# Jiahao-Ma/VFA

Hardware: AMD Instinct MI355X
Metric: voxels aggregated/sec (7 views->BEV grid) (higher is better)
Workload: dtype f32; 1 GPU; multiviewc_200x200x1; cameras_per_rank=7, cameras_total=7, channels=256, rccl_ranks=1, parallelism=single GPU

## Files before the change

vfa_amd/csrc/vfa_integral.hip:

```cpp
#include <hip/hip_runtime.h>
#include <stdint.h>

#include "../../include/vfa_hip.h"
#include "vfa_geom.h"
#include "vfa_split.h"

namespace {
using namespace vfa_dev;

constexpr int kMaxMaps = 4;
constexpr int kChunk = 32;

struct MapDesc {
    const float *feat;
    float *out;
    const float *scale;
    const float *shift;
    int H, W;
    unsigned row_blocks;
    unsigned long long col_vecs;
    unsigned *absmax;
};
struct MapArgs {
    MapDesc m[kMaxMaps];
    int n_maps, n_views, C;
};

template <bool AFFINE>
__global__ __launch_bounds__(kWave) void rows_batched_kernel(MapArgs a)
{
    __shared__ __align__(16) float tile[kWave][kChunk + 1];
    const int lane = threadIdx.x;
    unsigned b = blockIdx.x;
    int mi = 0;
    while (mi + 1 < a.n_maps && b >= a.m[mi].row_blocks) { b -= a.m[mi].row_blocks; ++mi; }
    const MapDesc &m = a.m[mi];
    const int H = m.H, W = m.W, C = a.C, cblocks = C / kWave;
    const int y = (int)(b % (unsigned)H);
    const unsigned rest = b / (unsigned)H;
    const int c0 = (int)(rest % (unsigned)cblocks) * kWave, v = (int)(rest / (unsigned)cblocks);
    const size_t plane = (size_t)H * W;
    const float *src = m.feat + ((size_t)v * C + c0) * plane + (size_t)y * W;
    float *dst = m.out + (((size_t)v * (H + 2) + (y + 1)) * (W + 2)) * C + c0;
    dst[lane] = 0.0f;
    dst[(size_t)(W + 1) * C + lane] = 0.0f;
    float sa = 1.0f, sb = 0.0f;
    if (AFFINE) {
        sa = m.scale[(size_t)v * C + c0 + lane];
        sb = m.shift[(size_t)v * C + c0 + lane];
    }
    auto act = [&](float x) {
        if (!AFFINE) return x;
        float t = x * sa;
        t = t + sb;
        return (t < 0.0f) ? 0.0f : t;
    };
    const int q = lane & 7, cq = lane & 15;
    double acc = 0.0;
    unsigned amax = 0u;
    for (int x0 = 0; x0 < W; x0 += kChunk) {
        const int nx = min(kChunk, W - x0);
        if (4 * q < nx) {
            for (int r = lane >> 3; r < kWave; r += 8) {
                const float4 t = *reinterpret_cast<const float4 *>(src + (size_t)r * plane + x0 + 4 * q);
                tile[r][4 * q + 0] = t.x; tile[r][4 * q + 1] = t.y; tile[r][4 * q + 2] = t.z; tile[r][4 * q + 3] = t.w;
            }
        }
        __syncthreads();
        for (int k = 0; k < nx; ++k) {
            const float f = act(tile[lane][k]);
            amax = max(amax, __float_as_uint(f) & 0x7fffffffu);
            acc += (double)f;
            tile[lane][k] = (float)acc;
        }
        __syncthreads();
        for (int k = lane >> 4; k < nx; k += 4) {
            const float4 t = make_float4(tile[4 * cq + 0][k], tile[4 * cq + 1][k], tile[4 * cq + 2][k], tile[4 * cq + 3][k]);
            *reinterpret_cast<float4 *>(dst + (size_t)(x0 + k + 1) * C + 4 * cq) = t;
        }
        __syncthreads();
    }
    if (m.absmax) {
        amax = wave_max_u32(amax);
        if (lane == 0) m.absmax[b] = amax;
    }
}

template <bool AFFINE>
__global__ __launch_bounds__(kWave) void rows_hwc_kernel(MapArgs a)
{
    const int lane = threadIdx.x;
    unsigned b = blockIdx.x;
    int mi = 0;
    while (mi + 1 < a.n_maps && b >= a.m[mi].row_blocks) { b -= a.m[mi].row_blocks; ++mi; }
    const MapDesc &m = a.m[mi];
    const int H = m.H, W = m.W, C = a.C, cblocks = C / kWave;
    const int y = (int)(b % (unsigned)H);
    const unsigned rest = b / (unsigned)H;
    const int c0 = (int)(rest % (unsigned)cblocks) * kWave, v = (int)(rest / (unsigned)cblocks);
    const float *src = m.feat + (((size_t)v * H + y) * W) * C + c0 + lane;
    float *dst = m.out + (((size_t)v * (H + 2) + (y + 1)) * (W + 2)) * C + c0 + lane;
    dst[0] = 0.0f;
    dst[(size_t)(W + 1) * C] = 0.0f;
    float sa = 1.0f, sb = 0.0f;
    if (AFFINE) {
        sa = m.scale[(size_t)v * C + c0 + lane];
        sb = m.shift[(size_t)v * C + c0 + lane];
    }
    auto act = [&](float x) {
        if (!AFFINE) return x;
        float t = x * sa;
        t = t + sb;
        return (t < 0.0f) ? 0.0f : t;
    };
    constexpr int U = 8;
    double acc = 0.0;
    unsigned amax = 0u;
    int x = 0;
    for (; x + U <= W; x += U) {
        float t[U];
#pragma unroll
        for (int k = 0; k < U; ++k) t[k] = src[(size_t)(x + k) * C];
#pragma unroll
        for (int k = 0; k < U; ++k) {
            const float f = act(t[k]);
            amax = max(amax, __float_as_uint(f) & 0x7fffffffu);
            acc += (double)f;
            dst[(size_t)(x + k + 1) * C] = (float)acc;
        }
    }
    for (; x < W; ++x) {
        const float f = act(src[(size_t)x * C]);
        amax = max(amax, __float_as_uint(f) & 0x7fffffffu);
        acc += (double)f;
        dst[(size_t)(x + 1) * C] = (float)acc;
    }
    if (m.absmax) {
        amax = wave_max_u32(amax);
        if (lane == 0) m.absmax[b] = amax;
    }
}

__global__ __launch_bounds__(256) void cols_batched_kernel(MapArgs a, unsigned long long total)
{
    unsigned long long i = (unsigned long long)blockIdx.x * 256 + threadIdx.x;
    if (i >= total) return;
    i = total - 1 - i;
    int mi = 0;
    while (mi + 1 < a.n_maps && i >= a.m[mi].col_vecs) { i -= a.m[mi].col_vecs; ++mi; }
    const MapDesc &m = a.m[mi];
    const int H = m.H;
    const size_t row_vecs = (size_t)(m.W + 2) * a.C / 4;
    const size_t v = i / row_vecs, r = i % row_vecs;
    float4 *p = reinterpret_cast<float4 *>(m.out) + v * (size_t)(H + 2) * row_vecs + r;
    const float4 zero = make_float4(0.f, 0.f, 0.f, 0.f);
    p[0] = zero;
    p[(size_t)(H + 1) * row_vecs] = zero;
    p += row_vecs;
    double a0 = 0.0, a1 = 0.0, a2 = 0.0, a3 = 0.0;
    auto step = [&](float4 &t) {
        a0 += (double)t.x; t.x = (float)a0;
        a1 += (double)t.y; t.y = (float)a1;
        a2 += (double)t.z; t.z = (float)a2;
        a3 += (double)t.w; t.w = (float)a3;
    };
    constexpr int U = 8;
    int y = 0;
    for (; y + U <= H; y += U) {
        float4 t[U];
#pragma unroll
        for (int k = 0; k < U; ++k) t[k] = p[(size_t)(y + k) * row_vecs];
#pragma unroll
        for (int k = 0; k < U; ++k) {
            step(t[k]);
            p[(size_t)(y + k) * row_vecs] = t[k];
        }
    }
    for (; y < H; ++y) {
        float4 t = p[(size_t)y * row_vecs];
        step(t);
        p[(size_t)y * row_vecs] = t;
    }
}

constexpr int kOpRows = 32, kOpCols = 32, kOpCh = 16, kOpThreads = kOpRows * kOpCh;
constexpr int kOpRowPitch = kOpCols * kOpCh + 16;
struct OnePassArgs {
    MapDesc m[kMaxMaps];
    unsigned unit_end[kMaxMaps];
    int split[kMaxMaps];
    int n_maps, n_views, C;
};
__device__ __forceinline__ void lds_barrier()
{
    asm volatile("s_waitcnt lgkmcnt(0)" ::: "memory");
    __builtin_amdgcn_s_barrier();
    asm volatile("" ::: "memory");
}
template <bool AFFINE>
__global__ __launch_bounds__(kOpThreads, 4) void integral_onepass_kernel(OnePassArgs a)
{
    extern __shared__ __align__(16) unsigned char op_lds[];
    float *tile = reinterpret_cast<float *>(op_lds);
    double *colacc = reinterpret_cast<double *>(op_lds + kOpRows * kOpRowPitch * 4);
    const int tid = threadIdx.x;
    unsigned u = blockIdx.x;
    int mi = 0;
    while (mi + 1 < a.n_maps && u >= a.unit_end[mi]) ++mi;
    if (mi > 0) u -= a.unit_end[mi - 1];
    const MapDesc &m = a.m[mi];
    const int H = m.H, W = m.W, C = a.C, cblocks = C / kOpCh;
    const int split = a.split[mi], part = split ? (int)(u & 1u) : 0;
    if (split) u >>= 1;
    const int v = (int)(u / (unsigned)cblocks), cb = (int)(u % (unsigned)cblocks), c0 = cb * kOpCh;
    const int r = tid >> 4, c = tid & 15;
    const size_t plane = (size_t)H * W;
    float *out_v = m.out + (size_t)v * (H + 2) * (W + 2) * C + c0;
    const int n_strips = (W + kOpCols - 1) / kOpCols;
    const int s_first = part ? split : 0, s_last = (split && !part) ? split : n_strips;
    const int xa = s_first * kOpCols, xb = min(W, s_last * kOpCols);
    {
        float *o = out_v + c;
        const int pa = part ? xa + 1 : 0, pb = (split && !part) ? xb + 1 : W + 2;
        for (int x = pa + r; x < pb; x += kOpRows) { o[(size_t)x * C] = 0.0f; o[((size_t)(H + 1) * (W + 2) + x) * C] = 0.0f; }
        for (int y = r; y < H; y += kOpRows) {
            if (!part) o[(size_t)(y + 1) * (W + 2) * C] = 0.0f;
            if (!split || part) o[((size_t)(y + 1) * (W + 2) + W + 1) * C] = 0.0f;
        }
    }
    for (int i = tid; i < (xb - xa) * kOpCh; i += kOpThreads) colacc[i] = 0.0;
    float sa = 1.0f, sb = 0.0f;
    if (AFFINE) { sa = m.scale[(size_t)v * C + c0 + c]; sb = m.shift[(size_t)v * C + c0 + c]; }
    auto act = [&](float x) {
        if (!AFFINE) return x;
        float t = x * sa;
        t = t + sb;
        return (t < 0.0f) ? 0.0f : t;
    };
    unsigned amax = 0u;
    auto load_strip = [&](float4 (&buf)[kOpCols / 4], int y0, int x0) {
        {
            const int x4 = tid & 7;
#pragma unroll
            for (int j = 0; j < kOpCols / 4; ++j) {
                const int line = (tid & ~63) + 8 * j + ((tid & 63) >> 3), row = line >> 4, ch = line & 15;
                buf[j] = *reinterpret_cast<const float4 *>(m.feat + ((size_t)v * C + c0 + ch) * plane + (size_t)min(y0 + row, H - 1) * W +
                                                           min(x0 + 4 * x4, W - 4));
            }
        }
    };
    float4 cur[kOpCols / 4];
    load_strip(cur, 0, 0);
    __syncthreads();
    bool stores_behind = false;
    for (int y0 = 0; y0 < H; y0 += kOpRows) {
        const int rows = min(kOpRows, H - y0);
        double racc = 0.0;
        for (int s = 0; s < s_last; ++s) {
            const int x0 = s * kOpCols, nx = min(kOpCols, W - x0);
            const bool carry_only = s < s_first;
            const bool last_strip = s + 1 == s_last;
            const bool more = !last_strip || y0 + kOpRows < H;
            if (stores_behind) __builtin_amdgcn_s_waitcnt(0x0f78);
            else __builtin_amdgcn_s_waitcnt(0x0f70);
            float *trow = tile + r * kOpRowPitch + c;
            {
                float *raw = tile;
#pragma unroll
                for (int j = 0; j < kOpCols / 4; ++j) {
                    float *p = raw + ((tid & ~63) + 8 * j + ((tid & 63) >> 3)) * 33 + 4 * (tid & 7);
                    p[0] = cur[j].x; p[1] = cur[j].y; p[2] = cur[j].z; p[3] = cur[j].w;
                }
#pragma unroll
                for (int j = 0; j < kOpCols / 4; ++j)
                    cur[j] = make_float4(raw[tid * 33 + 4 * j], raw[tid * 33 + 4 * j + 1], raw[tid * 33 + 4 * j + 2], raw[tid * 33 + 4 * j + 3]);
            }
            auto raw_of = [&](int k) {
                const float4 q = cur[k / 4];
                return (k & 3) == 0 ? q.x : (k & 3) == 1 ? q.y : (k & 3) == 2 ? q.z : q.w;
            };
            if (carry_only) {
                if (r < rows) {
#pragma unroll
                    for (int k = 0; k < kOpCols; ++k) racc += (double)act(raw_of(k));
                }
                if (more) load_strip(cur, last_strip ? y0 + kOpRows : y0, last_strip ? 0 : x0 + kOpCols);
                stores_behind = false;
                continue;
            }
            if (r < rows) {
                if (nx == kOpCols) {
#pragma unroll
                    for (int k = 0; k < kOpCols; ++k) {
                        const float f = act(raw_of(k));
                        amax = max(amax, __float_as_uint(f) & 0x7fffffffu);
                        racc += (double)f;
                        trow[k * kOpCh] = (float)racc;
                    }
                } else {
#pragma unroll
                    for (int k = 0; k < kOpCols; ++k) {
                        if (k < nx) {
                            const float f = act(raw_of(k));
                            amax = max(amax, __float_as_uint(f) & 0x7fffffffu);
                            racc += (double)f;
                            trow[k * kOpCh] = (float)racc;
                        }
                    }
                }
            }
            if (more) load_strip(cur, last_strip ? y0 + kOpRows : y0, last_strip ? 0 : x0 + kOpCols);
            lds_barrier();
            if (r < nx) {
                double acc = colacc[(x0 - xa + r) * kOpCh + c];
                float *tcol = tile + r * kOpCh + c;
                if (rows == kOpRows) {
#pragma unroll
                    for (int k = 0; k < kOpRows; ++k) {
                        acc += (double)tcol[k * kOpRowPitch];
                        tcol[k * kOpRowPitch] = (float)acc;
                    }
                } else {
                    for (int k = 0; k < rows; ++k) {
                        acc += (double)tcol[k * kOpRowPitch];
                        tcol[k * kOpRowPitch] = (float)acc;
                    }
                }
                colacc[(x0 - xa + r) * kOpCh + c] = acc;
            }
            lds_barrier();
#pragma unroll
            for (int j = 0; j < kOpCols / 4; ++j) {
                const int idx = tid + kOpThreads * j, row = min(idx >> 7, rows - 1), x = min((idx >> 2) & 31, nx - 1), c4 = idx & 3;
                *reinterpret_cast<float4 *>(out_v + ((size_t)(y0 + row + 1) * (W + 2) + (x0 + x + 1)) * C + 4 * c4) =
                    *reinterpret_cast<const float4 *>(tile + row * kOpRowPitch + x * kOpCh + 4 * c4);
            }
            stores_behind = more;
            lds_barrier();
        }
    }
    if (m.absmax) {
        __shared__ unsigned s_max[kOpThreads / kWave];
        amax = wave_max_u32(amax);
        if ((tid & 63) == 0) s_max[tid >> 6] = amax;
        __syncthreads();
        if (tid == 0) {
            unsigned mx = 0u;
            for (int k = 0; k < kOpThreads / kWave; ++k) mx = max(mx, s_max[k]);
            unsigned *e = m.absmax + ((size_t)v * (C / kWave) + (cb >> 2)) * H;
            const int q = 2 * (cb & 3) + part;
            for (int y = q; y < H; y += 8) e[y] = y == q ? mx : 0u;
            if (!split) for (int y = q + 1; y < H; y += 8) e[y] = 0u;
        }
    }
}

__global__ __launch_bounds__(kWave) void integral_absmax_kernel(const float *integral, unsigned *absmax, int n_views, int C, int H, int W,
                                                                unsigned units)
{
    const int lane = threadIdx.x, cblocks = (C + kWave - 1) / kWave;
    unsigned amax = 0u;
    for (unsigned b = blockIdx.x; b < units; b += gridDim.x) {
        const int y = (int)(b % (unsigned)H);
        const unsigned rest = b / (unsigned)H;
        const int c = (int)(rest % (unsigned)cblocks) * kWave + lane, v = (int)(rest / (unsigned)cblocks);
        if (c < C) {
            const float *up = integral + (((size_t)v * (H + 2) + y) * (W + 2)) * C + c, *dn = up + (size_t)(W + 2) * C;
            float u0 = up[0], d0 = dn[0];
            for (int x = 1; x <= W; ++x) {
                const float u1 = up[(size_t)x * C], d1 = dn[(size_t)x * C];
                const float f = ((d1 - u1) - d0) + u0;
                amax = max(amax, __float_as_uint(f) & 0x7fffffffu);
                u0 = u1; d0 = d1;
            }
        }
    }
    amax = wave_max_u32(amax);
    if (lane == 0) absmax[blockIdx.x] = amax;
}

bool aligned16(const void *p) { return (reinterpret_cast<uintptr_t>(p) & 15) == 0; }

}

namespace vfa_dev {
size_t feature_stats_count(int n_views, int C, int Hf)
{
    if (n_views < 0 || C <= 0 || Hf <= 0) return 0;
    return (size_t)n_views * Hf * ((C + kWave - 1) / kWave);
}
int integral_absmax_folded(const float *integral, unsigned *absmax, int n_views, int C, int Hf, int Wf, int max_entries, int *n_entries,
                               void *stream)
{
    const size_t n = feature_stats_count(n_views, C, Hf);
    if (!integral || !absmax || max_entries <= 0 || n == 0 || n >= (1ull << 31)) return VFA_ERR_BAD_ARGUMENT;
    const unsigned grid = n < (size_t)max_entries ? (unsigned)n : (unsigned)max_entries;
    hipLaunchKernelGGL(integral_absmax_kernel, dim3(grid), dim3(kWave), 0, (hipStream_t)stream, integral, absmax, n_views, C, Hf, Wf, (unsigned)n);
    *n_entries = (int)grid;
    return (int)hipGetLastError();
}

}

extern "C" {

static int integral_images_launch(const float *const *features, const float *const *scales, const float *const *shifts,
                                  float *const *integrals, unsigned *const *absmax, int n_views, int C, int n_maps, const int *feat_hw,
                                  bool hwc, void *stream)
{
    MapArgs a = {};
    a.n_maps = n_maps; a.n_views = n_views; a.C = C;
    unsigned long long row_blocks = 0, col_vecs = 0;
    for (int s = 0; s < n_maps; ++s) {
        MapDesc &m = a.m[s];
        m.feat = features[s]; m.out = integrals[s];
        m.scale = scales ? scales[s] : nullptr; m.shift = shifts ? shifts[s] : nullptr;
        m.absmax = absmax ? absmax[s] : nullptr;
        m.H = feat_hw[2 * s]; m.W = feat_hw[2 * s + 1];
        const unsigned long long rb = (unsigned long long)m.H * (C / kWave) * n_views;
        if (rb >= (1ull << 31)) return VFA_ERR_UNSUPPORTED;
        m.row_blocks = (unsigned)rb;
        m.col_vecs = (unsigned long long)n_views * (m.W + 2) * C / 4;
        row_blocks += rb; col_vecs += m.col_vecs;
    }
    if (row_blocks >= (1ull << 31) || (col_vecs + 255) / 256 >= (1ull << 31)) return VFA_ERR_UNSUPPORTED;
    hipStream_t st = (hipStream_t)stream;
    bool onepass = !hwc && C % kOpCh == 0 && C % kWave == 0 && (long long)n_views * (C / kOpCh) >= 64;
    int w_max = 0;
    for (int s = 0; s < n_maps && onepass; ++s) {
        onepass = a.m[s].H >= 8 && a.m[s].W >= 4 && (size_t)kOpRows * kOpRowPitch * 4 + (size_t)a.m[s].W * kOpCh * 8 <= 160 * 1024 - 1024;
        w_max = a.m[s].W > w_max ? a.m[s].W : w_max;
    }
    if (onepass) {
        OnePassArgs oa = {};
        oa.n_maps = n_maps; oa.n_views = n_views; oa.C = C;
        unsigned long long units = 0;
        for (int s = 0; s < n_maps; ++s) {
            oa.m[s] = a.m[s];
            const int n_strips = (a.m[s].W + kOpCols - 1) / kOpCols;
            oa.split[s] = n_strips >= 4 ? (6 * n_strips + 5) / 10 : 0;
            units += (unsigned long long)n_views * (C / kOpCh) * (oa.split[s] ? 2 : 1);
            oa.unit_end[s] = (unsigned)units;
        }
        if (units >= (1ull << 31)) return VFA_ERR_UNSUPPORTED;
        int part_max = 0;
        for (int s = 0; s < n_maps; ++s) {
            const int left = oa.split[s] * kOpCols, wide = oa.split[s] ? (left > a.m[s].W - left ? left : a.m[s].W - left) : a.m[s].W;
            part_max = wide > part_max ? wide : part_max;
        }
        const size_t lds = (size_t)kOpRows * kOpRowPitch * 4 + (size_t)part_max * kOpCh * 8;
        auto launch = [&](auto kern) {
            hipError_t e0 = hipFuncSetAttribute(reinterpret_cast<const void *>(kern), hipFuncAttributeMaxDynamicSharedMemorySize, (int)lds);
            if (e0 != hipSuccess) return (int)e0;
            hipLaunchKernelGGL(kern, dim3((unsigned)units), dim3(kOpThreads), lds, st, oa);
            return (int)hipGetLastError();
        };
        return scales ? launch(integral_onepass_kernel<true>) : launch(integral_onepass_kernel<false>);
    }
    if (hwc) {
        if (scales) hipLaunchKernelGGL((rows_hwc_kernel<true>), dim3((unsigned)row_blocks), dim3(kWave), 0, st, a);
        else hipLaunchKernelGGL((rows_hwc_kernel<false>), dim3((unsigned)row_blocks), dim3(kWave), 0, st, a);
    } else {
        if (scales) hipLaunchKernelGGL((rows_batched_kernel<true>), dim3((unsigned)row_blocks), dim3(kWave), 0, st, a);
        else hipLaunchKernelGGL((rows_batched_kernel<false>), dim3((unsigned)row_blocks), dim3(kWave), 0, st, a);
    }
    int e = (int)hipGetLastError();
    if (e) return e;
    hipLaunchKernelGGL(cols_batched_kernel, dim3((unsigned)((col_vecs + 255) / 256)), dim3(256), 0, st, a, col_vecs);
    return (int)hipGetLastError();
}

size_t vfa_feature_stats_count(int n_views, int C, int Hf) { return vfa_dev::feature_stats_count(n_views, C, Hf); }

int vfa_integral_absmax_f32(const float *integral, unsigned *absmax, int n_views, int C, int Hf, int Wf, void *stream)
{
    if (!integral || !absmax || n_views < 0 || C <= 0 || Hf <= 0 || Wf <= 0) return VFA_ERR_BAD_ARGUMENT;
    const size_t n = vfa_feature_stats_count(n_views, C, Hf);
    if (n == 0) return 0;
    if (n >= (1ull << 31)) return VFA_ERR_UNSUPPORTED;
    hipLaunchKernelGGL(integral_absmax_kernel, dim3((unsigned)n), dim3(kWave), 0, (hipStream_t)stream, integral, absmax, n_views, C, Hf, Wf,
                       (unsigned)n);
    return (int)hipGetLastError();
}

int vfa_integral_images_f32(const float *const *features, const float *const *scales, const float *const *shifts,
                            float *const *integrals, unsigned *const *absmax, int n_views, int C, int n_maps, const int *feat_hw,
                            void *stream)
{
    if (!features || !integrals || !feat_hw || n_views < 0 || C <= 0 || n_maps < 0) return VFA_ERR_BAD_ARGUMENT;
    if ((scales == nullptr) != (shifts == nullptr)) return VFA_ERR_BAD_ARGUMENT;
    for (int s = 0; s < n_maps; ++s) {
        if (feat_hw[2 * s] <= 0 || feat_hw[2 * s + 1] <= 0 || !features[s] || !integrals[s]) return VFA_ERR_BAD_ARGUMENT;
        if (scales && (!scales[s] || !shifts[s])) return VFA_ERR_BAD_ARGUMENT;
    }
    if (n_views == 0 || n_maps == 0) return 0;
    bool fast = (C % kWave == 0) && n_maps <= kMaxMaps;
    for (int s = 0; s < n_maps && fast; ++s)
        fast = (feat_hw[2 * s + 1] % 4 == 0) && aligned16(features[s]) && aligned16(integrals[s]);
    if (!fast) {
        for (int s = 0; s < n_maps; ++s) {
            const int st = scales ? vfa_affine_relu_integral_image_f32(features[s], scales[s], shifts[s], integrals[s], n_views, C,
                                                                        feat_hw[2 * s], feat_hw[2 * s + 1], stream)
                                  : vfa_integral_image_f32(features[s], integrals[s], n_views, C, feat_hw[2 * s], feat_hw[2 * s + 1], stream);
            if (st) return st;
            if (absmax && absmax[s]) {
                const int st2 = vfa_integral_absmax_f32(integrals[s], absmax[s], n_views, C, feat_hw[2 * s], feat_hw[2 * s + 1], stream);
                if (st2) return st2;
            }
        }
        return 0;
    }
    return integral_images_launch(features, scales, shifts, integrals, absmax, n_views, C, n_maps, feat_hw, false, stream);
}

int vfa_integral_images_hwc_f32(const float *const *features_hwc, const float *const *scales, const float *const *shifts,
                                float *const *integrals, unsigned *const *absmax, int n_views, int C, int n_maps, const int *feat_hw,
                                void *stream)
{
    if (!features_hwc || !integrals || !feat_hw || n_views < 0 || C <= 0 || n_maps < 0) return VFA_ERR_BAD_ARGUMENT;
    if ((scales == nullptr) != (shifts == nullptr)) return VFA_ERR_BAD_ARGUMENT;
    for (int s = 0; s < n_maps; ++s) {
        if (feat_hw[2 * s] <= 0 || feat_hw[2 * s + 1] <= 0 || !features_hwc[s] || !integrals[s]) return VFA_ERR_BAD_ARGUMENT;
        if (scales && (!scales[s] || !shifts[s])) return VFA_ERR_BAD_ARGUMENT;
    }
    if (n_views == 0 || n_maps == 0) return 0;
    if (C % kWave != 0 || n_maps > kMaxMaps) return VFA_ERR_UNSUPPORTED;
    for (int s = 0; s < n_maps; ++s)
        if (!aligned16(integrals[s])) return VFA_ERR_UNSUPPORTED;
    return integral_images_launch(features_hwc, scales, shifts, integrals, absmax, n_views, C, n_maps, feat_hw, true, stream);
}

}
```

Baseline: 1.529 billion voxels/s.

## Double-buffer strip loads via inline asm and batch LDS column scans in one-pass kernel

Restructures the one-pass integral kernel so each strip's global loads for the next strip are issued at the start, into a second register buffer, using inline asm global_load_dwordx4. This lets the loads overlap the current strip's transpose and scan work. The column scan prefetches LDS values in batches of eight, and the output stores are grouped four at a time with scheduling barriers. Occupancy hints drop from 4 to 2 blocks, and dynamic LDS is padded to at least 81KB, which appears to force lower occupancy deliberately. The trade-off is more register pressure and fewer resident blocks in exchange for more latency hiding.

Measured after the change: 1.528 billion voxels/s, median of 2. About the same (-0.1%).

```diff
diff --git a/vfa_amd/csrc/vfa_integral.hip b/vfa_amd/csrc/vfa_integral.hip
--- a/vfa_amd/csrc/vfa_integral.hip
+++ b/vfa_amd/csrc/vfa_integral.hip
@@ -184,7 +184,9 @@
 }
 
 constexpr int kOpRows = 32, kOpCols = 32, kOpCh = 16, kOpThreads = kOpRows * kOpCh;
+constexpr int kColBatch = 8;
 constexpr int kOpRowPitch = kOpCols * kOpCh + 16;
+typedef float strip_regs __attribute__((ext_vector_type(4)));
 struct OnePassArgs {
     MapDesc m[kMaxMaps];
     unsigned unit_end[kMaxMaps];
@@ -198,7 +200,7 @@
     asm volatile("" ::: "memory");
 }
 template <bool AFFINE>
-__global__ __launch_bounds__(kOpThreads, 4) void integral_onepass_kernel(OnePassArgs a)
+__global__ __launch_bounds__(kOpThreads, 2) void integral_onepass_kernel(OnePassArgs a)
 {
     extern __shared__ __align__(16) unsigned char op_lds[];
     float *tile = reinterpret_cast<float *>(op_lds);
@@ -238,31 +240,34 @@
         return (t < 0.0f) ? 0.0f : t;
     };
     unsigned amax = 0u;
-    auto load_strip = [&](float4 (&buf)[kOpCols / 4], int y0, int x0) {
+    auto load_strip = [&](strip_regs (&buf)[kOpCols / 4], int y0, int x0) {
         {
             const int x4 = tid & 7;
 #pragma unroll
             for (int j = 0; j < kOpCols / 4; ++j) {
                 const int line = (tid & ~63) + 8 * j + ((tid & 63) >> 3), row = line >> 4, ch = line & 15;
-                buf[j] = *reinterpret_cast<const float4 *>(m.feat + ((size_t)v * C + c0 + ch) * plane + (size_t)min(y0 + row, H - 1) * W +
-                                                           min(x0 + 4 * x4, W - 4));
+                const float *src = m.feat + ((size_t)v * C + c0 + ch) * plane + (size_t)min(y0 + row, H - 1) * W +
+                                   min(x0 + 4 * x4, W - 4);
+                asm volatile("global_load_dwordx4 %0, %1, off" : "=v"(buf[j]) : "v"(src) : "memory");
             }
         }
     };
-    float4 cur[kOpCols / 4];
-    load_strip(cur, 0, 0);
+    strip_regs buf_a[kOpCols / 4], buf_b[kOpCols / 4];
+    load_strip(buf_a, 0, 0);
     __syncthreads();
     bool stores_behind = false;
-    for (int y0 = 0; y0 < H; y0 += kOpRows) {
-        const int rows = min(kOpRows, H - y0);
-        double racc = 0.0;
-        for (int s = 0; s < s_last; ++s) {
+    double racc = 0.0;
+    auto strip = [&](strip_regs (&cur)[kOpCols / 4], strip_regs (&nxt)[kOpCols / 4], int y0, int s) __attribute__((always_inline)) {
+            const int rows = min(kOpRows, H - y0);
+            if (s == 0) racc = 0.0;
             const int x0 = s * kOpCols, nx = min(kOpCols, W - x0);
             const bool carry_only = s < s_first;
             const bool last_strip = s + 1 == s_last;
             const bool more = !last_strip || y0 + kOpRows < H;
             if (stores_behind) __builtin_amdgcn_s_waitcnt(0x0f78);
             else __builtin_amdgcn_s_waitcnt(0x0f70);
+            __builtin_amdgcn_sched_barrier(0);
+            if (more) load_strip(nxt, last_strip ? y0 + kOpRows : y0, last_strip ? 0 : x0 + kOpCols);
             float *trow = tile + r * kOpRowPitch + c;
             {
                 float *raw = tile;
@@ -273,10 +278,10 @@
                 }
 #pragma unroll
                 for (int j = 0; j < kOpCols / 4; ++j)
-                    cur[j] = make_float4(raw[tid * 33 + 4 * j], raw[tid * 33 + 4 * j + 1], raw[tid * 33 + 4 * j + 2], raw[tid * 33 + 4 * j + 3]);
+                    cur[j] = strip_regs{raw[tid * 33 + 4 * j], raw[tid * 33 + 4 * j + 1], raw[tid * 33 + 4 * j + 2], raw[tid * 33 + 4 * j + 3]};
             }
             auto raw_of = [&](int k) {
-                const float4 q = cur[k / 4];
+                const strip_regs q = cur[k / 4];
                 return (k & 3) == 0 ? q.x : (k & 3) == 1 ? q.y : (k & 3) == 2 ? q.z : q.w;
             };
             if (carry_only) {
@@ -284,9 +289,8 @@
 #pragma unroll
                     for (int k = 0; k < kOpCols; ++k) racc += (double)act(raw_of(k));
                 }
-                if (more) load_strip(cur, last_strip ? y0 + kOpRows : y0, last_strip ? 0 : x0 + kOpCols);
                 stores_behind = false;
-                continue;
+                return;
             }
             if (r < rows) {
                 if (nx == kOpCols) {
@@ -309,34 +313,62 @@
                     }
                 }
             }
-            if (more) load_strip(cur, last_strip ? y0 + kOpRows : y0, last_strip ? 0 : x0 + kOpCols);
             lds_barrier();
             if (r < nx) {
                 double acc = colacc[(x0 - xa + r) * kOpCh + c];
                 float *tcol = tile + r * kOpCh + c;
-                if (rows == kOpRows) {
-#pragma unroll
-                    for (int k = 0; k < kOpRows; ++k) {
-                        acc += (double)tcol[k * kOpRowPitch];
-                        tcol[k * kOpRowPitch] = (float)acc;
-                    }
-                } else {
-                    for (int k = 0; k < rows; ++k) {
-                        acc += (double)tcol[k * kOpRowPitch];
-                        tcol[k * kOpRowPitch] = (float)acc;
+                const int n_groups = (rows + kColBatch - 1) / kColBatch;
+                float t[kColBatch];
+#pragma unroll
+                for (int j = 0; j < kColBatch; ++j) t[j] = tcol[j * kOpRowPitch];
+                __builtin_amdgcn_sched_barrier(0);
+#pragma unroll
+                for (int g = 0; g < kOpRows / kColBatch; ++g) {
+                    if (g + 1 < n_groups) {
+#pragma unroll
+                        for (int j = 0; j < kColBatch; ++j) {
+                            acc += (double)t[j];
+                            tcol[(g * kColBatch + j) * kOpRowPitch] = (float)acc;
+                            t[j] = tcol[((g + 1) * kColBatch + j) * kOpRowPitch];
+                            __builtin_amdgcn_sched_barrier(0);
+                        }
+                    } else {
+#pragma unroll
+                        for (int j = 0; j < kColBatch; ++j) {
+                            acc += (double)t[j];
+                            tcol[(g * kColBatch + j) * kOpRowPitch] = (float)acc;
+                            __builtin_amdgcn_sched_barrier(0);
+                        }
+                        break;
                     }
                 }
                 colacc[(x0 - xa + r) * kOpCh + c] = acc;
             }
             lds_barrier();
-#pragma unroll
-            for (int j = 0; j < kOpCols / 4; ++j) {
+            auto tile_piece = [&](int j, float4 *&dst) {
                 const int idx = tid + kOpThreads * j, row = min(idx >> 7, rows - 1), x = min((idx >> 2) & 31, nx - 1), c4 = idx & 3;
-                *reinterpret_cast<float4 *>(out_v + ((size_t)(y0 + row + 1) * (W + 2) + (x0 + x + 1)) * C + 4 * c4) =
-                    *reinterpret_cast<const float4 *>(tile + row * kOpRowPitch + x * kOpCh + 4 * c4);
+                dst = reinterpret_cast<float4 *>(out_v + ((size_t)(y0 + row + 1) * (W + 2) + (x0 + x + 1)) * C + 4 * c4);
+                return *reinterpret_cast<const float4 *>(tile + row * kOpRowPitch + x * kOpCh + 4 * c4);
+            };
+#pragma unroll
+            for (int j0 = 0; j0 < kOpCols / 4; j0 += 4) {
+                float4 *d0, *d1, *d2, *d3;
+                const float4 q0 = tile_piece(j0, d0), q1 = tile_piece(j0 + 1, d1), q2 = tile_piece(j0 + 2, d2), q3 = tile_piece(j0 + 3, d3);
+                __builtin_amdgcn_sched_barrier(0);
+                *d0 = q0; *d1 = q1; *d2 = q2; *d3 = q3;
+                __builtin_amdgcn_sched_barrier(0);
             }
             stores_behind = more;
             lds_barrier();
+    };
+    {
+        const int total = ((H + kOpRows - 1) / kOpRows) * s_last;
+        int y0 = 0, s = 0;
+        auto advance = [&]() { if (++s == s_last) { s = 0; y0 += kOpRows; } };
+        for (int t = 0; t < total; t += 2) {
+            strip(buf_a, buf_b, y0, s);
+            advance();
+            if (t + 1 < total) { strip(buf_b, buf_a, y0, s); advance(); }
         }
     }
     if (m.absmax) {
@@ -448,7 +480,8 @@
             const int left = oa.split[s] * kOpCols, wide = oa.split[s] ? (left > a.m[s].W - left ? left : a.m[s].W - left) : a.m[s].W;
             part_max = wide > part_max ? wide : part_max;
         }
-        const size_t lds = (size_t)kOpRows * kOpRowPitch * 4 + (size_t)part_max * kOpCh * 8;
+        size_t lds = (size_t)kOpRows * kOpRowPitch * 4 + (size_t)part_max * kOpCh * 8;
+        if (lds < 81 * 1024) lds = 81 * 1024;
         auto launch = [&](auto kern) {
             hipError_t e0 = hipFuncSetAttribute(reinterpret_cast<const void *>(kern), hipFuncAttributeMaxDynamicSharedMemorySize, (int)lds);
             if (e0 != hipSuccess) return (int)e0;
```
